# lokyhark/spalinalg

Hardware: AMD Instinct MI355X
Metric: CSR SpMV GFLOP/s (f64, 10Mx10M, 140M nnz) (higher is better)
Workload: dtype f64

## Files before the change

spalinalg_amd/csrc/csr_slide.hpp:

```cpp
#pragma once
#include "csr_kernels.hpp"

namespace spal {

constexpr uint32_t kSlideAsync = 1u << 16;
constexpr uint32_t kSlideAsyncVecs = 1;
#ifndef SPAL_SLIDE_FIRST_BATCH
#define SPAL_SLIDE_FIRST_BATCH 12
#endif
constexpr uint32_t kSlideFirstBatch = SPAL_SLIDE_FIRST_BATCH;

template <typename T>
struct SlideVec { using type = __attribute__((ext_vector_type(4))) uint32_t; };

template <typename T>
__device__ __forceinline__ typename SlideVec<T>::type slide_load_vec(const T *__restrict__ x, uint32_t page, uint32_t v,
                                                                      uint32_t last_vec) {
    using vec_t = typename SlideVec<T>::type;
    constexpr uint32_t VP = kPageCols / (16 / sizeof(T));
    return reinterpret_cast<const vec_t *>(x)[min(page * VP + v, last_vec)];
}

template <typename T>
__device__ __forceinline__ typename SlideVec<T>::type slide_load_vec_tail(const T *__restrict__ x, uint32_t page, uint32_t v,
// ... 11 lines not shown
}

struct SlideNew { uint32_t lo0, lo1, hi0, hi1; };
__device__ __forceinline__ SlideNew slide_new_pages(uint32_t fa, uint32_t na, uint32_t fb, uint32_t nb) {
    const uint32_t ea = fa + na, eb = fb + nb;
    SlideNew r;
    if (fa >= eb || ea <= fb) {
        r.lo0 = fb; r.lo1 = eb; r.hi0 = eb; r.hi1 = eb;
        return r;
    }
    r.lo0 = fb; r.lo1 = max(fb, min(fa, eb));
    r.hi0 = min(eb, max(ea, fb)); r.hi1 = eb;
    return r;
}

template <typename T, int RPT, int S, bool UNI>
__device__ __forceinline__ void slide_tile_load(StreamTile<T> &t, const uint32_t *__restrict__ rowptr,
                                                const uint16_t *__restrict__ col16, const T *__restrict__ vals,
                                                uint32_t row0, uint32_t nrows, uint32_t b, uint32_t e, uint32_t lane,
                                                uint32_t ulen) {
    using pair_t = typename Pair<T>::type;
    static_assert(RPT <= 64, "a row per lane");
    const uint32_t rlast = min(row0 + (uint32_t)RPT, nrows);
    t.start = b & ~1u;
    t.steps = (e - t.start + 127u) >> 7;
    const uint32_t e0 = t.start + lane * 2;
    const uint32_t jmax = max(t.steps, 1u) - 1u;
#pragma unroll
    for (int j = 0; j < S; ++j) {
        const uint32_t at = e0 + min((uint32_t)j, jmax) * 128u;
        t.v[j] = __builtin_nontemporal_load(reinterpret_cast<const pair_t *>(vals + at));
        t.c[j] = __builtin_nontemporal_load(reinterpret_cast<const uint32_t *>(col16 + at));
    }
    if constexpr (UNI) {
        const uint32_t len = ulen - 1u, nrt = rlast - min(row0, rlast);
        t.rp0 = b + min(lane, nrt) * len;
        t.rp1 = b + min(lane + 1u, nrt) * len;
    } else {
        t.rp0 = rowptr[min(row0 + lane, rlast)];
        t.rp1 = rowptr[min(row0 + lane + 1u, rlast)];
    }
}

template <typename T, int RPT, int S, bool UNI, int PF>
__global__ __launch_bounds__(kStreamBlock, 2) void csr_spmv_slide(
    const uint32_t *__restrict__ rowptr, const uint16_t *__restrict__ col16, const T *__restrict__ vals,
    const T *__restrict__ x, T *__restrict__ y, const uint2 *__restrict__ sdesc, uint32_t nrows, uint32_t ncols,
    uint32_t nsteps, uint32_t per_xcd, uint32_t chunk, uint32_t NP, uint32_t ulen, uint32_t flags) {
    static_assert(PF == 1 || PF == 2, "one or two tiles of loads ahead");
    static_assert(S >= 1 && S <= kStreamSteps, "a tile holds at most kStreamSteps steps");
    using vec_t = typename SlideVec<T>::type;
    extern __shared__ __attribute__((aligned(16))) unsigned char spal_smem[];
    constexpr uint32_t V = 16 / sizeof(T), VP = kPageCols / V;
    constexpr int NB = PF + 1;
    const bool nt_store = flags & 1u;
    T *prod_all = reinterpret_cast<T *>(spal_smem);
    T *xw = prod_all + kStreamWaves * stream_strip<false>();
    vec_t *xw4 = reinterpret_cast<vec_t *>(xw);

    const uint32_t xcd = blockIdx.x & 7u, slot = blockIdx.x >> 3, slots = gridDim.x >> 3;
    const bool even = flags & 8u;
    const uint32_t xbase = even ? xcd * (nsteps / 8u) + min(xcd, nsteps % 8u) : xcd * per_xcd;
    if (xbase >= nsteps) return;
    const uint32_t nx = even ? nsteps / 8u + (xcd < nsteps % 8u ? 1u : 0u) : min(per_xcd, nsteps - xbase);
    if (nx == 0u) return;
// ... 18 lines not shown
    const bool arith = UNI && (flags & 4u);
    auto tile_b = [&](uint32_t k) { const uint32_t r = min(tile_row(k), nrows); return arith ? r * (ulen - 1u) : rowptr[r]; };
    auto tile_e = [&](uint32_t k) { const uint32_t r = min(tile_row(k) + (uint32_t)RPT, nrows); return arith ? r * (ulen - 1u) : rowptr[r]; };

    StreamTile<T> t[NB];
    uint32_t tb[NB], te[NB];
#pragma unroll
    for (int q = 0; q < NB; ++q) {
        tb[q] = tile_b((uint32_t)q);
        te[q] = tile_e((uint32_t)q);
    }
    uint2 d = sdesc[gi(0u)];
    uint2 dn = sdesc[gi(1u)];
#pragma unroll
    for (int q = 0; q < PF; ++q)
        slide_tile_load<T, RPT, S, UNI>(t[q], rowptr, col16, vals, tile_row((uint32_t)q), nrows, tb[q], te[q], lane, ulen);
    {
        const uint32_t f = d.x, nv = (d.y & 0xffu) * VP;
        for (uint32_t j0 = threadIdx.x; j0 < nv; j0 += kSlideFirstBatch * kStreamBlock) {
            vec_t r[kSlideFirstBatch];
#pragma unroll
            for (uint32_t k = 0; k < kSlideFirstBatch; ++k) {
                const uint32_t j = min(j0 + k * kStreamBlock, nv - 1u);
                r[k] = slide_load_vec_tail<T>(x, f + j / VP, j % VP, ncols);
            }
#pragma unroll
            for (uint32_t k = 0; k < kSlideFirstBatch; ++k) {
                const uint32_t j = j0 + k * kStreamBlock;
                if (j < nv) xw4[((f + j / VP) % NP) * VP + j % VP] = r[k];
            }
        }
// ... 5 lines not shown
        constexpr int KN = (K + PF) % NB;
        const uint32_t skip = (d.y >> 8) & 0xfu;
        const bool more = i + 1u < nk;
        SlideNew nw = slide_new_pages(d.x, d.y & 0xffu, dn.x, dn.y & 0xffu);
        const uint32_t nlo = (nw.lo1 - nw.lo0) * VP;
        const uint32_t ntot = more ? nlo + (nw.hi1 - nw.hi0) * VP : 0u;
        const bool async = more && (dn.y & kSlideAsync) && (even || (i + 1u) % chunk != 0u);
        auto new_page = [&](uint32_t j) { return j < nlo ? nw.lo0 + j / VP : nw.hi0 + (j - nlo) / VP; };
        vec_t nv[kSlideAsyncVecs];
#pragma unroll
        for (uint32_t k = 0; k < kSlideAsyncVecs; ++k) {
            const uint32_t j = threadIdx.x + k * kStreamBlock;
            const bool mine = async && j < ntot;
            nv[k] = slide_load_vec<T>(x, mine ? new_page(j) : 0u, mine ? j % VP : 0u, last_vec);
        }
        slide_tile_load<T, RPT, S, UNI>(t[KN], rowptr, col16, vals, tile_row(i + PF), nrows, tb[KN], te[KN], lane, ulen);
        tb[K] = tile_b(i + PF + 1u);
        te[K] = tile_e(i + PF + 1u);
        const uint32_t r0 = (gi(i) * kStreamWaves + wave) * (uint32_t)RPT;
#ifdef SPAL_DIAG
        if (SPAL_DIAG_ON(flags, 11)) {
            T sacc = T(0);
#pragma unroll
            for (int j = 0; j < S; ++j) sacc += t[K].v[j].x + t[K].v[j].y + T(t[K].c[j]);
            if (r0 + lane < nrows) y[r0 + lane] = sacc + T(t[K].rp1 - t[K].rp0);
        } else
#endif
        if (r0 < nrows && !((skip >> wave) & 1u)) {
            stream_compute<T, RPT, false>(t[K], xw, wmax, prod, y, r0, nrows, lane, nt_store, flags);
        } else if (r0 < nrows && ((d.y >> (20u + wave)) & 1u)) {
            const uint32_t re = min(r0 + (uint32_t)RPT, nrows), rm = min(r0 + (uint32_t)RPT / 2u, re);
            const uint32_t eb = rowptr[r0], em = rowptr[rm], ee = rowptr[re];
            slide_tile_load<T, RPT, S, false>(t[K], rowptr, col16, vals, r0, rm, eb, em, lane, 0u);
            stream_compute<T, RPT, false>(t[K], xw, wmax, prod, y, r0, rm, lane, nt_store, flags);
            if (rm < re) {
                __builtin_amdgcn_wave_barrier();
                slide_tile_load<T, RPT, S, false>(t[K], rowptr, col16, vals, rm, re, em, ee, lane, 0u);
                stream_compute<T, RPT, false>(t[K], xw, wmax, prod, y, rm, re, lane, nt_store, flags);
            }
        }
#pragma unroll
        for (uint32_t k = 0; k < kSlideAsyncVecs; ++k) {
            const uint32_t j = threadIdx.x + k * kStreamBlock;
            if (async && j < ntot) xw4[(new_page(j) % NP) * VP + j % VP] = nv[k];
        }
// ... 31 lines not shown
```

spalinalg_amd/csrc/spal_csr.hip:

```cpp
#include "csr_kernels.hpp"
#include "csr_slide.hpp"
#include "spal_ops.hpp"

namespace spal {

template <typename K>
static hipError_t raise_lds_cap(K kern, int device, size_t lds, std::atomic<uint64_t> &configured) {
    if (lds <= 48 * 1024) return hipSuccess;
    const uint64_t bit = 1ull << (device & 63);
    if (configured.load(std::memory_order_relaxed) & bit) return hipSuccess;
    hipError_t e = hipFuncSetAttribute((const void *)kern, hipFuncAttributeMaxDynamicSharedMemorySize,
                                       160 * 1024);
    if (e == hipSuccess) configured.fetch_or(bit, std::memory_order_relaxed);
    return e;
}

template <typename T, int L, int U, bool LDSX, int BLOCK, int LB = 1>
static hipError_t launch_vec(const spal_csr *a, const void *x, void *y, hipStream_t st) {
    const CsrPlan &p = a->plan;
    const uint32_t per_xcd = (p.nblocks + 7) / 8;
    const size_t lds = LDSX ? (size_t)p.lds_entries * sizeof(T) : 0;
    auto kern = csr_spmv_vector<T, L, U, LDSX, true, BLOCK, LB>;
    static std::atomic<uint64_t> configured{0};
    hipError_t e = raise_lds_cap(kern, a->device, lds, configured);
// ... 231 lines not shown
    const hipError_t e = typed([&](auto t) { return launch_lanes<decltype(t)>(a, x_dev, y_dev, stream); });
    if (e != hipSuccess)
        return fail(SPAL_ERR_HIP, "csr spmv launch failed: %s", hipGetErrorString(e));
    return SPAL_OK;
}

void csr_free(spal_csr *a) {
    if (!a) return;
    for (spal_csr *part : a->parts) csr_free(part);
    (void)dev_free(a->d_rowptr);
    (void)dev_free(a->d_colind);
    (void)dev_free(a->d_values);
    (void)dev_free(a->d_desc);
    if (a->col16_placed) place_free(a->device, a->d_col16);
    else (void)dev_free(a->d_col16);
    (void)dev_free(a->d_pages);
    (void)dev_free(a->d_ovtiles);
    (void)dev_free(a->d_sdesc);
    (void)dev_free(a->d_ovtiles_slide);
    (void)dev_free(a->d_ptiles);
    (void)dev_free(a->d_pwin);
    if (a->split_short) csr_free(a->split_short);
    (void)dev_free(a->d_split_rows);
    blockwin_free(a);
    if (a->d_vec_block && a->vec_block_owned) (void)hipFree(a->d_vec_block);
    else place_free(a->device, a->d_vec_block);
    (void)dev_free(a->d_win_groups);
    cblock_free(a);
    trsv_free(a);
    trsv_sweep_free(a);
// ... 288 lines not shown
    {"stream_global", &CsrPlan::stream_global, 0, 1, nullptr, "stream_global must be 0 or 1"},
    {"window_pages", &CsrPlan::window_pages, 0, 64, nullptr, "window_pages must be in [0, 64]"},
    {"col16", &CsrPlan::vec_col16_allowed, 0, 1, nullptr, "col16 must be 0 or 1"},
    {"stream_row_max", &CsrPlan::stream_row_max, 1, 1024, nullptr, "stream_row_max must be in [1, 1024]"},
    {"nt_store", &CsrPlan::nt_store, 0, 1, nullptr, "nt_store must be 0 or 1"},
    {"persistent_blocks", &CsrPlan::persistent_blocks, 0, 4096, [](int64_t v) { return v == 0 || (v >= 8 && v % 8 == 0); },
     "persistent_blocks must be 0 (auto) or a multiple of 8 in [8, 4096]"},
    {"slide", &CsrPlan::slide_user, -1, 1, nullptr, "slide must be -1 (auto), 0 or 1"},
    {"panel_pages", &CsrPlan::panel_pages, 0, 255, nullptr, "panel_pages must be in [0, 255]"},
    {"panel_window", &CsrPlan::panel_window_user, 0, 624, nullptr, "panel_window must be in [0, 624] pages"},
    {"panel_on", &CsrPlan::panel_on, 0, 1, nullptr, "panel_on must be 0 or 1"},
    {"slide_run", &CsrPlan::slide_run, 0, 65535, nullptr, "slide_run must be in [0, 65535]"},
    {"slide_even", &CsrPlan::slide_even, 0, 1, nullptr, "slide_even must be 0 or 1"},
    {"arith_bounds", &CsrPlan::arith_bounds, 0, 1, nullptr, "arith_bounds must be 0 or 1"},
    {"split_tiles", &CsrPlan::split_tiles_on, 0, 1, nullptr, "split_tiles must be 0 or 1"},
    {"place_tries", &CsrPlan::place_tries, 0, 16, nullptr, "place_tries must be in [0, 16]"},
    {"uniform_rows", &CsrPlan::uniform_rows, 0, 1, nullptr, "uniform_rows must be 0 or 1"},
    {"prefetch", &CsrPlan::prefetch, 1, 2, nullptr, "prefetch must be 1 or 2"},
    {"xcd_chunk", &CsrPlan::xcd_chunk, 0, 4096, nullptr, "xcd_chunk must be in [0, 4096]"},
    {"cblock_rows", &CsrPlan::cblock_rows_user, 0, 8192, nullptr,
     "cblock_rows (rows of a row block of the column-blocked kernel) must be 0 (auto) or in [1, 8192]"},
    {"cblock_shift", &CsrPlan::cblock_shift_user, 0, 24, [](int64_t v) { return v == 0 || v >= 8; },
     "cblock_shift (log2 of the columns of a column block) must be 0 (auto: 2 MB of x) or in [8, 24]"},
    {"cblock_form", &CsrPlan::cblock_form_user, -1, 1, nullptr, "cblock_form must be -1 (auto), 0 (entry-parallel) or 1 (rows form)"},
};

int spal_csr_set_option(spal_csr_t a, const char *key, int64_t value) {
    if (!a || !key) return fail(SPAL_ERR_INVALID_ARGUMENT, "spal_csr_set_option: null argument");
    {
        int st = SPAL_OK;
// ... 180 lines not shown
             (p.kernel == 2 && p.persistent && p.tiles_per_wave == 4) ? 1 : 0,
             p.kernel == 2 ? p.nt_store : 0, p.kernel == 2 ? p.uniform_row_fraction : 0.0,
             p.kernel == 2 ? p.prefetch : 0, (p.kernel == 2 && p.slide && p.slide_on && p.slide_fill_ok) ? 1 : 0,
             p.kernel == 2 ? p.ring_pages : 0, (p.kernel == 2 && p.slide) ? p.slide_S : 0,
             (p.kernel == 2 && p.slide && p.slide_on) ? a->n_split_tiles : 0u,
             (p.kernel == 2 && p.panel_on) ? a->n_ptiles : 0u,
             (double)a->tuned_us[0], (double)a->tuned_us[1],
             (double)a->tuned_us[2], (double)a->tuned_us[3], (double)a->place_us[0], (double)a->place_us[1],
             a->place_tried, (unsigned long long)(uintptr_t)a->d_values,
             (unsigned long long)(uintptr_t)a->d_col16, (unsigned long long)(uintptr_t)a->d_rowptr,
             (double)a->walk_us[0], (double)a->walk_us[1], a->walk_blocks, a->walk_probes, place_block_count(a->device),
             (unsigned long long)place_free_bytes(a->device),
             p.kernel == 2 ? p.nonlocal_row_fraction : 0.0, (p.cblock && p.cblock_on) ? 1 : 0, p.cblock_pending, p.cblock ? p.cblock_rows : 0, !p.cblock ? "" : p.cblock_form ? "rows" : "entry", p.cblock ? (double)p.cblock_run : 0.0,
             p.cblock ? (1ull << p.cblock_shift) : 0ull, p.cblock ? p.cblock_nbc : 0, p.cblock ? p.cblock_nrb : 0u,
             (double)a->cblock_us[0], (double)a->cblock_us[1], a->cblock_failed);
    return SPAL_OK;
}
int spal_csr_describe(spal_csr_t a, char *buf, size_t buf_len) {
    if (!a || !buf || !buf_len) return fail(SPAL_ERR_INVALID_ARGUMENT, "spal_csr_describe: null argument");
    SPAL_TRY(csr_describe_plan(a, buf, buf_len));
    return ops_describe_append(buf, buf_len, a->ops, a);
}

}
```

spalinalg_amd/csrc/spal_csr_plan.hip:

```cpp
#include "csr_kernels.hpp"
#include "spal_internal.hpp"

namespace spal {

__global__ __launch_bounds__(256) void csr_block_windows(
    const uint32_t *__restrict__ rowptr, const uint32_t *__restrict__ colind, uint32_t nrows,
    uint32_t R, uint2 *__restrict__ out) {
    __shared__ uint32_t s_min, s_max;
    if (threadIdx.x == 0) {
        s_min = 0xffffffffu;
        s_max = 0u;
    }
    __syncthreads();
    const uint32_t row0 = blockIdx.x * R;
    const uint32_t row1 = min(row0 + R, nrows);
    uint32_t lo = 0xffffffffu, hi = 0u;
    for (uint32_t r = row0 + threadIdx.x; r < row1; r += 256) {
        const uint32_t a0 = rowptr[r], a1 = rowptr[r + 1];
        if (a0 < a1) {
            lo = min(lo, colind[a0]);
            hi = max(hi, colind[a1 - 1] + 1u);
        }
    }
    atomicMin(&s_min, lo);
// ... 425 lines not shown
        }
    }
    CsrPlan &p = a->plan;
    const double mean = a->nrows ? (double)a->nnz / (double)a->nrows : 0.0;
    if (!p.user_lanes) p.lanes_per_row = mean > 85.0 ? 64 : mean > 64.0 ? 32 : pick_lanes(mean);
    p.long_rows = mean > 64.0 ? 1 : 0;
    if (!p.user_unroll) p.unroll = mean > 64.0 ? 1 : 4;
    if (!p.user_threads) p.threads = 1024;
    if (a->d_desc) {
        SPAL_HIP_TRY(dev_free(a->d_desc));
        a->d_desc = nullptr;
    }
    p.stream_row_fraction = 0.0;
    p.vec_col16 = 0;
    p.slide = 0;
    p.ring_pages = 0;
    if (a->nnz == 0) {
        cblock_free(a);
        p.kernel = 1;
        p.rows_per_block = 1024;
        p.nblocks = (uint32_t)((a->nrows + 1023) / 1024);
        p.lds_x = 0;
        return SPAL_OK;
    }
    const uint32_t valign = 16u / (uint32_t)a->elem_size;

    if ((p.user_kernel == 0 && mean <= 120.0) || p.user_kernel == 2) {
        if (p.tiles_per_wave != 4 && p.tiles_per_wave != 8) p.tiles_per_wave = 4;
        const int rpt_all[] = {256, 128, 64, 32, 24, 16, 12, 8};
        std::vector<int> rpts;
// ... 87 lines not shown
            for (uint32_t b = 0; b < p.nblocks && !any_stream; ++b) any_stream = best_desc[b].z == kModeStream;
            if (any_stream || a->n_ptiles) {
                if (!a->d_col16) {
                    SPAL_HIP_TRY(dev_alloc((void **)&a->d_col16, (size_t)a->cap_entries * sizeof(uint16_t)));
                    SPAL_HIP_TRY(hipMemsetAsync(a->d_col16, 0, (size_t)a->cap_entries * sizeof(uint16_t), a->stream));
                }
                if (any_stream)
                    hipLaunchKernelGGL(csr_encode_col16, dim3(p.nblocks), dim3(256), 0, a->stream, a->d_rowptr,
                                       a->d_colind, a->d_desc, a->d_pages, a->d_col16, (uint32_t)a->nrows, R,
                                       (uint32_t)p.ring_pages);
                if (a->n_ptiles)
                    hipLaunchKernelGGL(csr_encode_col16_span, dim3(a->n_ptiles), dim3(256), 0, a->stream, a->d_rowptr,
                                       a->d_colind, a->d_ptiles, a->d_pwin, a->d_col16, (uint32_t)a->nrows, R);
                SPAL_HIP_TRY(hipGetLastError());
            }
            if (best_over) {
                uint32_t *d_list = nullptr;
                const uint32_t pieces = (uint32_t)std::max(1, best_rpt / 64) * best_over;
                SPAL_HIP_TRY(dev_alloc((void **)&d_list, ((size_t)pieces + 1) * 4));
                a->d_ovtiles = d_list;
                SPAL_HIP_TRY(hipMemsetAsync(d_list, 0, 4, a->stream));
                const uint64_t ntile = (a->nrows + (uint64_t)best_rpt - 1) / (uint64_t)best_rpt;
                hipLaunchKernelGGL(csr_overflow_tiles, dim3((uint32_t)((ntile + 255) / 256)), dim3(256), 0, a->stream,
                                   a->d_desc, (uint32_t)a->nrows, R, (uint32_t)best_rpt, pieces, d_list,
                                   d_list + 1);
                SPAL_HIP_TRY(hipGetLastError());
                uint32_t listed = 0;
                SPAL_HIP_TRY(hipMemcpyAsync(&listed, d_list, 4, hipMemcpyDeviceToHost, a->stream));
                SPAL_HIP_TRY(hipStreamSynchronize(a->stream));
                if (listed > pieces || listed < best_over)
// ... 9 lines not shown
                p.nonlocal_row_fraction = (double)far_rows / (double)a->nrows;
                p.cblock_pending = 0;
                if (getenv("SPAL_CBLOCK_DEBUG"))
                    fprintf(stderr, "[spal cblock] plan: nonlocal rows %.3f, user %d, lazy %d\n", p.nonlocal_row_fraction, p.cblock_user, a->cblock_lazy);
                if (p.cblock_user == 1 || (p.cblock_user < 0 && p.nonlocal_row_fraction >= 0.5)) {
                    if (a->cblock_lazy && p.cblock_user < 0) { cblock_free(a); p.cblock_pending = 1; }
                    else (void)cblock_plan(a, p.cblock_user == 1);
                } else {
                    cblock_free(a);
                }
            }
            return SPAL_OK;
        }
    }
    cblock_free(a);

    p.kernel = 1;
    if (p.threads != 512 && p.threads != 1024) p.threads = 1024;
    const uint32_t budget = kLdsBudgetBytes / (uint32_t)a->elem_size;
    const uint32_t cand_all[] = {4096, 2048, 1024, 512};
    std::vector<uint32_t> cands;
    if (p.user_rows_per_block) {
        cands.push_back((uint32_t)p.rows_per_block);
    } else if (mean > 64.0) {
        uint32_t r0 = 1024;
        while (r0 > 64 && (double)r0 * mean > 131072.0) r0 >>= 1;
        if (p.threads == 1024) {
            const double want = std::max(1.0, (double)a->nnz / 100000.0);
            const uint64_t rounds = std::max<uint64_t>(1, (uint64_t)(want / 512.0 + 0.5));
            const uint64_t nb = rounds * 502;
// ... 71 lines not shown
```

spalinalg_amd/csrc/spal_csr_slide.hip:

```cpp
#include "csr_panel.hpp"
#include "csr_slide.hpp"
#include "spal_internal.hpp"

namespace spal {

template <typename T, int RPT, int S, bool UNI>
static hipError_t launch_slide_inst(const spal_csr *a, const void *x, void *y, hipStream_t st) {
    constexpr int PF = 2;
    const CsrPlan &p = a->plan;
    const size_t lds = ((size_t)kStreamWaves * stream_strip<false>() + (size_t)p.ring_pages * kPageCols) * sizeof(T);
    const int per_cu = (int)std::min<size_t>(8, std::max<size_t>(1, (160 * 1024) / (lds + 512)));
    const uint32_t grid = p.persistent_blocks > 0 ? (uint32_t)p.persistent_blocks : 256u * (uint32_t)per_cu;
    const uint32_t per_xcd = (p.slide_steps + 7u) / 8u;
    const uint32_t slots = std::max(1u, grid / 8u);
    const uint32_t one_run = (per_xcd + slots - 1u) / slots;
    const uint32_t chunk = p.slide_run > 0 ? std::min<uint32_t>((uint32_t)p.slide_run, one_run) : one_run;
    const bool even = p.slide_run <= 0 && p.slide_even;
    const uint32_t used = even ? std::min(slots, per_xcd) : std::min(slots, (per_xcd + chunk - 1u) / chunk);
    auto kern = csr_spmv_slide<T, RPT, S, UNI, PF>;
    static std::atomic<uint64_t> configured{0};
    const uint64_t bit = 1ull << (a->device & 63);
    if (lds > 48 * 1024 && !(configured.load(std::memory_order_relaxed) & bit)) {
        hipError_t e = hipFuncSetAttribute((const void *)kern, hipFuncAttributeMaxDynamicSharedMemorySize, 160 * 1024);
        if (e != hipSuccess) return e;
        configured.fetch_or(bit, std::memory_order_relaxed);
    }
    hipLaunchKernelGGL(kern, dim3(used * 8u), dim3(kStreamBlock), lds, st, a->d_rowptr, a->d_col16,
                       (const T *)a->d_values, (const T *)x, (T *)y, a->d_sdesc, (uint32_t)a->nrows, (uint32_t)a->ncols,
                       p.slide_steps, per_xcd, chunk, (uint32_t)p.ring_pages, (uint32_t)p.slide_uniform,
                       (uint32_t)(p.nt_store ? 1 : 0) | (uint32_t)p.diag | ((UNI && p.all_rows_uniform && p.arith_bounds) ? 4u : 0u) | (even ? 8u : 0u));
    return hipGetLastError();
}

template <typename T, int RPT, bool UNI>
static hipError_t launch_slide_steps(const spal_csr *a, const void *x, void *y, hipStream_t st) {
    switch (std::max(4, a->plan.slide_S)) {
        case 4: return launch_slide_inst<T, RPT, 4, UNI>(a, x, y, st);
        case 5: return launch_slide_inst<T, RPT, 5, UNI>(a, x, y, st);
        case 6: return launch_slide_inst<T, RPT, 6, UNI>(a, x, y, st);
        case 7: return launch_slide_inst<T, RPT, 7, UNI>(a, x, y, st);
        case 8: return launch_slide_inst<T, RPT, 8, UNI>(a, x, y, st);
        default: return hipErrorInvalidValue;
// ... 7 lines not shown
}

template <typename T>
static hipError_t launch_slide_rpt(const spal_csr *a, const void *x, void *y, hipStream_t st) {
    switch (a->plan.rows_per_tile) {
        case 64: return launch_slide_uni<T, 64>(a, x, y, st);
        case 32: return launch_slide_uni<T, 32>(a, x, y, st);
        case 24: return launch_slide_uni<T, 24>(a, x, y, st);
        case 16: return launch_slide_uni<T, 16>(a, x, y, st);
        case 12: return launch_slide_uni<T, 12>(a, x, y, st);
        case 8: return launch_slide_uni<T, 8>(a, x, y, st);
        default: return hipErrorInvalidValue;
    }
}

hipError_t launch_slide(const spal_csr *a, const void *x, void *y, hipStream_t st) {
    return a->elem_size == 8 ? launch_slide_rpt<double>(a, x, y, st) : launch_slide_rpt<float>(a, x, y, st);
}

template <typename T, int RPT>
static hipError_t launch_panel_inst(const spal_csr *a, const void *x, void *y, hipStream_t st) {
    const CsrPlan &p = a->plan;
    const size_t lds = std::max((size_t)kStreamWaves * stream_strip<false>(), (size_t)p.panel_window_pages * kPageCols) * sizeof(T);
    auto kern = csr_spmv_panel<T, RPT>;
    static std::atomic<uint64_t> configured{0};
    const uint64_t bit = 1ull << (a->device & 63);
    if (lds > 48 * 1024 && !(configured.load(std::memory_order_relaxed) & bit)) {
        hipError_t e = hipFuncSetAttribute((const void *)kern, hipFuncAttributeMaxDynamicSharedMemorySize, 160 * 1024);
        if (e != hipSuccess) return e;
        configured.fetch_or(bit, std::memory_order_relaxed);
    }
// ... 142 lines not shown
    p.slide = 1;
    p.ring_pages = (int)NP;
    p.slide_steps = nsteps;
    p.slide_S = (int)S;
    p.slide_uniform = (uni && ulen != 0u) ? (int)ulen : 0;
    {
        const double tiles = (double)nsteps * kStreamWaves;
        const double avg_steps = tiles > 0 ? (double)a->nnz / tiles / 128.0 : 0.0;
        p.slide_fill_ok = (p.slide_fill_user >= 0) ? p.slide_fill_user : (avg_steps >= 0.6 * (double)std::max(4u, S) ? 1 : 0);
    }
    p.all_rows_uniform = (p.slide_uniform && left_over.empty() && n_split == 0 &&
                          (uint64_t)a->nrows * (uint64_t)(ulen - 1u) == a->nnz) ? 1 : 0;
    return SPAL_OK;
}

}
```

spalinalg_amd/csrc/spal_csr_tune.hip:

```cpp
#include "spal_internal.hpp"

namespace spal {

template <typename T>
static int csr_autotune(spal_csr_t a, const T *x_dev, T *y_dev, void *stream, int iters) {
    if (!a) return fail(SPAL_ERR_INVALID_ARGUMENT, "spal_csr_autotune: handle is NULL");
    if (a->elem_size != (int)sizeof(T))
        return fail(SPAL_ERR_INVALID_ARGUMENT, "spal_csr_autotune: handle holds %s values",
                    a->elem_size == 8 ? "f64" : "f32");
    if (!x_dev || !y_dev) return fail(SPAL_ERR_INVALID_ARGUMENT, "spal_csr_autotune: null vector");
    if (!a->parts.empty()) {
        for (size_t b = 0; b < a->parts.size(); ++b)
            SPAL_TRY(csr_autotune<T>(a->parts[b], x_dev, y_dev + a->part_row0[b], stream, iters));
        return SPAL_OK;
    }
    if (iters < 1) iters = 1;
    DeviceGuard guard(a->device);
    if (guard.status != SPAL_OK) return guard.status;
    SPAL_TRY(csr_ensure_plan(a, nullptr, false));
    if (a->bw_on) return SPAL_OK;
    if (a->split_short) return csr_autotune<T>(a->split_short, x_dev, y_dev, stream, iters);
    std::lock_guard<std::mutex> lock(a->mu);
    CsrPlan &p = a->plan;
    for (float &t : a->tuned_us) t = 0.f;
// ... 38 lines not shown
            p.nt_store = (cand >> 1) & 1;
            float ms = 0.f;
            timed(iters, &ms);
            if (rc == SPAL_OK && round == 1) {
                a->tuned_us[cand] = ms * 1e3f;
                if (ms < best_ms) { best_ms = ms; best = cand; }
                if (cand == planned) planned_ms = ms;
            }
        }
    }
    if (planned_ms <= 1.01f * best_ms) best = planned;
    if (walking_is_slide) { p.slide_on = best & 1; p.slide_fill_ok = 1; p.persistent = 0; }
    else p.persistent = best & 1;
    p.user_persistent = true;
    p.nt_store = (best >> 1) & 1;
    int tries = p.place_tries;
    if (const char *e = getenv("SPAL_PLACE_TRIES")) tries = atoi(e);
    const size_t cbytes = a->d_col16 ? (size_t)a->cap_entries * sizeof(uint16_t) : 0;
    if (rc == SPAL_OK && tries > 0 && cbytes >= ((size_t)64 << 20) && !a->col16_placed) {
        const int n = std::max(4, iters / 4);
        float cur_ms = 0.f;
        timed(n, &cur_ms);
        a->place_us[0] = cur_ms * 1e3f;
        uint16_t *const original = a->d_col16;
        std::vector<void *> cand;
        std::vector<float> ms_of;
        const int kept = place_block_count(a->device);
        for (int k = 0; k < kept && k < tries && rc == SPAL_OK; ++k) {
            void *b = place_alloc(a->device, k, cbytes);
            if (!b) continue;
            hipError_t e = hipMemcpyAsync(b, original, cbytes, hipMemcpyDeviceToDevice, st);
            if (e != hipSuccess) { place_free(a->device, b); rc = fail(SPAL_ERR_HIP, "spal_csr_autotune: %s", hipGetErrorString(e)); break; }
            a->d_col16 = (uint16_t *)b;
            float ms = 0.f;
            timed(n, &ms);
            cand.push_back(b); ms_of.push_back(ms);
            ++a->place_tried;
        }
        int best = -1;
        for (size_t k = 0; k < ms_of.size(); ++k)
            if (ms_of[k] < 0.99f * cur_ms && (best < 0 || ms_of[k] < ms_of[(size_t)best])) best = (int)k;
        (void)hipStreamSynchronize(st);
        a->d_col16 = best >= 0 ? (uint16_t *)cand[(size_t)best] : original;
        for (size_t k = 0; k < cand.size(); ++k)
            if ((int)k != best) place_free(a->device, cand[k]);
        if (best >= 0) { (void)dev_free(original); a->col16_placed = 1; }
        a->place_us[1] = (best >= 0 ? ms_of[(size_t)best] : cur_ms) * 1e3f;
    }
    return rc;
}

}

using namespace spal;

extern "C" {

int spal_csr_alloc_vectors(spal_csr_t a, void **x_dev, void **y_dev, void *stream) {
    if (!a || !x_dev || !y_dev) return fail(SPAL_ERR_INVALID_ARGUMENT, "spal_csr_alloc_vectors: null argument");
    DeviceGuard guard(a->device);
    if (guard.status != SPAL_OK) return guard.status;
// ... 127 lines not shown
```

spalinalg_amd/csrc/spal_internal.hpp:

```cpp
#pragma once

#include <hip/hip_runtime.h>
#include <stdint.h>

#include <algorithm>
#include <atomic>
#include <cstdarg>
#include <cstdio>
#include <cstring>
#include <functional>
#include <mutex>
#include <string>
#include <thread>
#include <vector>

#include "../../include/spal.h"

namespace spal {

std::string &last_error_ref();
int fail(int status, const char *fmt, ...) __attribute__((format(printf, 2, 3)));

#define SPAL_HIP_TRY(expr)                                                          \
    do {                                                                            \
// ... 155 lines not shown
    int cblock_rows_user = 0, cblock_shift_user = 0;
    int cblock_form_user = -1;
    int cblock_form = 0;
    float cblock_run = 0.f;
    int cblock_shift = 0;
    int cblock_nbc = 0;
    uint32_t cblock_nrb = 0;
    double nonlocal_row_fraction = 0.0;
    int slide_S = 0;
    int slide_uniform = 0;
    int all_rows_uniform = 0;
    int arith_bounds = 1;
    int slide_fill_ok = 1;
    int slide_fill_user = -1;
    int slide_even = 1;
    int blockwin = -1;
    int row_split = -1;
    int split_threshold = 128;
    int place_tries = 8;
    int split_tiles_on = 1;
    int diag = 0;
    int persistent_blocks = 0;
    int rows_per_block = 0;
    int lds_x = 0;
    uint32_t lds_entries = 0;
    uint32_t nblocks = 0;
    double lds_row_fraction = 0.0;
    double stream_row_fraction = 0.0;
    double uniform_row_fraction = 0.0;
    bool user_rows_per_block = false, user_lanes = false, user_lds = false,
// ... 86 lines not shown
    uint32_t bw_blocks = 0, bw_rows = 0, bw_cols = 0, bw_grid = 0;
    uint32_t bw_list_rows = 0;
    int bw_on = 0;
    float bw_us[2] = {0.f, 0.f};
    int plan_pending = 0;
    int cblock_lazy = 0;
    int cblock_failed = 0;
    void *d_vec_block = nullptr;
    int vec_block_owned = 0;
    size_t vec_x_off = 0, vec_y_off = 0;
    float walk_us[2] = {0.f, 0.f};
    int walk_blocks = 0;
    int walk_probes = 0;
    int walk_max = 8;
    int col16_placed = 0;
    std::mutex mu_cb;
    float tuned_us[4] = {0.f, 0.f, 0.f, 0.f};
    float place_us[2] = {0.f, 0.f};
    int place_tried = 0;
    spal::CsrPlan plan;
    std::vector<uint2> win_base;
    uint2 *d_win_groups = nullptr;
    uint32_t win_groups = 0, win_group_bits = 0;
    std::mutex mu;
    void *d_x = nullptr, *d_y = nullptr;
    hipStream_t stream = nullptr;
    std::vector<spal_csr *> parts;
    std::vector<uint64_t> part_row0, part_entry0;
    spal::OpState ops;
    uint64_t spmm_last = 0;
// ... 90 lines not shown
namespace spal {
int csr_plan_build(spal_csr *a);
constexpr uint32_t kWinBase = 256;
int csr_try_row_split(spal_csr *a, bool *did);
int csr_blockwin_or_split(spal_csr *a);
int csr_launch(spal_csr *a, const void *x_dev, void *y_dev, hipStream_t stream);
int csr_launch_planned(spal_csr *a, const void *x_dev, void *y_dev, hipStream_t stream);
int csr_ensure_plan(spal_csr *a, hipStream_t launch_stream, bool from_launch);
void csr_free(spal_csr *a);
int spmm_launch(spal_csr *a, int tile, uint64_t k, const void *x_dev, uint64_t ldx, void *y_dev, uint64_t ldy,
                hipStream_t stream);
void trsv_free(spal_csr *a);
void trsv_sweep_free(spal_csr *a);
hipError_t launch_slide(const spal_csr *a, const void *x, void *y, hipStream_t st);
int slide_plan(spal_csr *a, uint32_t rpt, const std::vector<uint4> &desc, const std::vector<uint32_t> &skip, uint32_t super_pages);
hipError_t launch_panel(const spal_csr *a, const void *x, void *y, hipStream_t st);
int csc_plan_build(spal_csc *a);
constexpr uint32_t kCscModeGlobal = 0, kCscModeLds = 1;
constexpr uint32_t kCscChunk = 1024;
hipError_t launch_csc_scatter(spal_csc *a, const void *x, void *y, hipStream_t st);
uint32_t csc_window_budget(const spal_csc *a, int cols);
size_t csc_scatter_lds_bytes(const spal_csc *a);
int csc_scatter_per_cu(const spal_csc *a);
bool csc_gave_up_consume(spal_csc *a);
int csc_invalid_products(const spal_csc *a);
int csc_rowtiles_plan(spal_csc *a);
void csc_rowtiles_free(spal_csc *a);
hipError_t launch_csc_rowtiles(const spal_csc *a, const void *x, void *y, hipStream_t st);
int cblock_plan(spal_csr *a, bool force);
void cblock_free(spal_csr *a);
// ... 11 lines not shown
```

Measured before the change: 1158.

## Compress uniform-row column indices into packed per-row delta records for slide SpMV

For matrices whose rows all have the same even length (12–16), each row's ring-relative column positions are encoded at plan time as a base plus byte deltas and a high-bit mask in 5–6 dwords per row. The slide kernel loads these records instead of the 16-bit column array, then decodes them in registers and transposes them through LDS into the usual tile column layout. This is meant to cut column-index traffic, roughly 24 bytes per row instead of 28–32, since SpMV is bandwidth bound. In exchange it adds decode ALU work, extra LDS round-trips and wave barriers per tile, plus build and verify kernels at planning time. The path is auto-enabled and then kept or dropped by an autotune timing comparison.

```diff
diff --git a/spalinalg_amd/csrc/csr_rowrec.hpp b/spalinalg_amd/csrc/csr_rowrec.hpp
--- /dev/null
+++ b/spalinalg_amd/csrc/csr_rowrec.hpp
@@ -0,0 +1,101 @@
+#pragma once
+#include <stdint.h>
+
+#if defined(__HIPCC__)
+#define SPAL_ROWREC_HD __host__ __device__ __forceinline__
+#else
+#define SPAL_ROWREC_HD inline
+#endif
+
+namespace spal {
+
+constexpr int kRowrecMinLen = 12, kRowrecMaxLen = 16;
+constexpr int kRowrecHighBits = 40;
+constexpr int kRowrecMaxDwords = 6;
+constexpr int rowrec_dwords(int L) { return L <= 14 ? 5 : 6; }
+constexpr bool rowrec_length_ok(int L) { return L >= kRowrecMinLen && L <= kRowrecMaxLen && L % 2 == 0; }
+constexpr uint32_t rowrec_max_span(int L, uint32_t R) {
+    const uint32_t by_bits = ((uint32_t)(kRowrecHighBits - 1 - (L - 2)) << 8) | 255u;
+    return R == 0u ? 0u : (by_bits < R - 1u ? by_bits : R - 1u);
+}
+
+template <int L>
+SPAL_ROWREC_HD void rowrec_pad(uint32_t *rec) {
+    const uint64_t H = (1ull << (L - 1)) - 1ull;
+    rec[0] = (uint32_t)(H << 16);
+    rec[1] = (uint32_t)(H >> 16);
+    for (int q = 2; q < rowrec_dwords(L); ++q) rec[q] = 0u;
+}
+
+template <int L>
+SPAL_ROWREC_HD bool rowrec_encode(const uint32_t *cols, uint32_t R, uint32_t *rec) {
+    static_assert(L >= 2 && L - 1 <= kRowrecHighBits && 7 + L - 1 <= 4 * kRowrecMaxDwords, "the record's fields");
+    constexpr int NR = rowrec_dwords(L);
+    for (int k = 1; k < L; ++k)
+        if (cols[k] <= cols[k - 1]) return false;
+    const uint32_t span = cols[L - 1] - cols[0];
+    if (R == 0u || R > 65536u || span >= R || (span >> 8) + (uint32_t)(L - 2) > (uint32_t)(kRowrecHighBits - 1)) return false;
+    uint64_t H = 0;
+    uint32_t w[kRowrecMaxDwords] = {0u, 0u, 0u, 0u, 0u, 0u};
+    for (int k = 1; k < L; ++k) {
+        const uint32_t d = cols[k] - cols[0];
+        H |= 1ull << ((d >> 8) + (uint32_t)(k - 1));
+        const int byte = 7 + (k - 1);
+        w[byte >> 2] |= (d & 255u) << (8 * (byte & 3));
+    }
+    w[0] |= (cols[0] % R) | (uint32_t)(H << 16);
+    w[1] |= (uint32_t)(H >> 16);
+    for (int q = 0; q < NR; ++q) rec[q] = w[q];
+    return true;
+}
+
+template <int L>
+SPAL_ROWREC_HD void rowrec_decode(const uint32_t *rec, uint32_t R, uint32_t *pos) {
+    const uint32_t base = rec[0] & 0xffffu;
+    uint64_t H = (uint64_t)(rec[0] >> 16) | ((uint64_t)(rec[1] & 0xffffffu) << 16);
+    pos[0] = base;
+#if defined(__clang__)
+#pragma unroll
+#endif
+    for (int k = 1; k < L; ++k) {
+        const uint32_t b = (uint32_t)__builtin_ctzll(H | (1ull << kRowrecHighBits));
+        H &= H - 1ull;
+        const int byte = 7 + (k - 1);
+        const uint32_t low = (rec[byte >> 2] >> (8 * (byte & 3))) & 255u;
+        const uint32_t p = base + (((b - (uint32_t)(k - 1)) << 8) | low);
+        pos[k] = p >= R ? p - R : p;
+    }
+}
+
+}
+
+#if defined(__HIPCC__)
+#include "csr_kernels.hpp"
+
+namespace spal {
+
+template <typename T, int L>
+__device__ __forceinline__ void rowrec_tile_load(StreamTile<T> &t, const uint32_t *__restrict__ rec, uint32_t tix,
+                                                 uint32_t lane) {
+    constexpr int NR = rowrec_dwords(L);
+    const uint32_t *at = rec + (size_t)tix * (NR * 64u) + lane;
+#pragma unroll
+    for (int q = 0; q < NR; ++q) t.c[q] = __builtin_nontemporal_load(at + q * 64);
+}
+
+template <typename T, int L>
+__device__ __forceinline__ void rowrec_expand(StreamTile<T> &t, uint32_t *strip, uint32_t R, uint32_t lane) {
+    static_assert(L % 2 == 0 && L / 2 <= kStreamSteps && 64 * (L / 2) * 4 <= kStreamTileNnz * (int)sizeof(T), "the strip holds the tile");
+    uint32_t pos[L];
+    rowrec_decode<L>(t.c, R, pos);
+    __builtin_amdgcn_wave_barrier();
+#pragma unroll
+    for (int i = 0; i < L / 2; ++i) strip[(L / 2) * lane + i] = pos[2 * i] | (pos[2 * i + 1] << 16);
+    __builtin_amdgcn_wave_barrier();
+#pragma unroll
+    for (int j = 0; j < L / 2; ++j) t.c[j] = strip[j * 64 + lane];
+    __builtin_amdgcn_wave_barrier();
+}
+
+}
+#endif
diff --git a/spalinalg_amd/csrc/csr_slide.hpp b/spalinalg_amd/csrc/csr_slide.hpp
--- a/spalinalg_amd/csrc/csr_slide.hpp
+++ b/spalinalg_amd/csrc/csr_slide.hpp
@@ -1,5 +1,6 @@
 #pragma once
 #include "csr_kernels.hpp"
+#include "csr_rowrec.hpp"
 
 namespace spal {
 
@@ -49,7 +50,7 @@
     return r;
 }
 
-template <typename T, int RPT, int S, bool UNI>
+template <typename T, int RPT, int S, bool UNI, int REC = 0>
 __device__ __forceinline__ void slide_tile_load(StreamTile<T> &t, const uint32_t *__restrict__ rowptr,
                                                 const uint16_t *__restrict__ col16, const T *__restrict__ vals,
                                                 uint32_t row0, uint32_t nrows, uint32_t b, uint32_t e, uint32_t lane,
@@ -61,11 +62,12 @@
     t.steps = (e - t.start + 127u) >> 7;
     const uint32_t e0 = t.start + lane * 2;
     const uint32_t jmax = max(t.steps, 1u) - 1u;
+    if constexpr (REC != 0) rowrec_tile_load<T, REC>(t, reinterpret_cast<const uint32_t *>(col16), row0 / 64u, lane);
 #pragma unroll
     for (int j = 0; j < S; ++j) {
         const uint32_t at = e0 + min((uint32_t)j, jmax) * 128u;
         t.v[j] = __builtin_nontemporal_load(reinterpret_cast<const pair_t *>(vals + at));
-        t.c[j] = __builtin_nontemporal_load(reinterpret_cast<const uint32_t *>(col16 + at));
+        if constexpr (REC == 0) t.c[j] = __builtin_nontemporal_load(reinterpret_cast<const uint32_t *>(col16 + at));
     }
     if constexpr (UNI) {
         const uint32_t len = ulen - 1u, nrt = rlast - min(row0, rlast);
@@ -77,13 +79,14 @@
     }
 }
 
-template <typename T, int RPT, int S, bool UNI, int PF>
+template <typename T, int RPT, int S, bool UNI, int PF, int REC = 0>
 __global__ __launch_bounds__(kStreamBlock, 2) void csr_spmv_slide(
     const uint32_t *__restrict__ rowptr, const uint16_t *__restrict__ col16, const T *__restrict__ vals,
     const T *__restrict__ x, T *__restrict__ y, const uint2 *__restrict__ sdesc, uint32_t nrows, uint32_t ncols,
     uint32_t nsteps, uint32_t per_xcd, uint32_t chunk, uint32_t NP, uint32_t ulen, uint32_t flags) {
     static_assert(PF == 1 || PF == 2, "one or two tiles of loads ahead");
     static_assert(S >= 1 && S <= kStreamSteps, "a tile holds at most kStreamSteps steps");
+    static_assert(REC == 0 || (UNI && RPT == 64 && rowrec_length_ok(REC) && S == REC / 2), "row records: uniform rows, a row per lane");
     using vec_t = typename SlideVec<T>::type;
     extern __shared__ __attribute__((aligned(16))) unsigned char spal_smem[];
     constexpr uint32_t V = 16 / sizeof(T), VP = kPageCols / V;
@@ -132,7 +135,7 @@
     uint2 dn = sdesc[gi(1u)];
 #pragma unroll
     for (int q = 0; q < PF; ++q)
-        slide_tile_load<T, RPT, S, UNI>(t[q], rowptr, col16, vals, tile_row((uint32_t)q), nrows, tb[q], te[q], lane, ulen);
+        slide_tile_load<T, RPT, S, UNI, REC>(t[q], rowptr, col16, vals, tile_row((uint32_t)q), nrows, tb[q], te[q], lane, ulen);
     {
         const uint32_t f = d.x, nv = (d.y & 0xffu) * VP;
         for (uint32_t j0 = threadIdx.x; j0 < nv; j0 += kSlideFirstBatch * kStreamBlock) {
@@ -168,7 +171,7 @@
             const bool mine = async && j < ntot;
             nv[k] = slide_load_vec<T>(x, mine ? new_page(j) : 0u, mine ? j % VP : 0u, last_vec);
         }
-        slide_tile_load<T, RPT, S, UNI>(t[KN], rowptr, col16, vals, tile_row(i + PF), nrows, tb[KN], te[KN], lane, ulen);
+        slide_tile_load<T, RPT, S, UNI, REC>(t[KN], rowptr, col16, vals, tile_row(i + PF), nrows, tb[KN], te[KN], lane, ulen);
         tb[K] = tile_b(i + PF + 1u);
         te[K] = tile_e(i + PF + 1u);
         const uint32_t r0 = (gi(i) * kStreamWaves + wave) * (uint32_t)RPT;
@@ -181,8 +184,9 @@
         } else
 #endif
         if (r0 < nrows && !((skip >> wave) & 1u)) {
+            if constexpr (REC != 0) rowrec_expand<T, REC>(t[K], reinterpret_cast<uint32_t *>(prod), NP * kPageCols, lane);
             stream_compute<T, RPT, false>(t[K], xw, wmax, prod, y, r0, nrows, lane, nt_store, flags);
-        } else if (r0 < nrows && ((d.y >> (20u + wave)) & 1u)) {
+        } else if (REC == 0 && r0 < nrows && ((d.y >> (20u + wave)) & 1u)) {
             const uint32_t re = min(r0 + (uint32_t)RPT, nrows), rm = min(r0 + (uint32_t)RPT / 2u, re);
             const uint32_t eb = rowptr[r0], em = rowptr[rm], ee = rowptr[re];
             slide_tile_load<T, RPT, S, false>(t[K], rowptr, col16, vals, r0, rm, eb, em, lane, 0u);
diff --git a/spalinalg_amd/csrc/spal_csr.hip b/spalinalg_amd/csrc/spal_csr.hip
--- a/spalinalg_amd/csrc/spal_csr.hip
+++ b/spalinalg_amd/csrc/spal_csr.hip
@@ -269,6 +269,7 @@
     (void)dev_free(a->d_desc);
     if (a->col16_placed) place_free(a->device, a->d_col16);
     else (void)dev_free(a->d_col16);
+    rowrec_free(a);
     (void)dev_free(a->d_pages);
     (void)dev_free(a->d_ovtiles);
     (void)dev_free(a->d_sdesc);
@@ -587,6 +588,8 @@
     {"slide_even", &CsrPlan::slide_even, 0, 1, nullptr, "slide_even must be 0 or 1"},
     {"arith_bounds", &CsrPlan::arith_bounds, 0, 1, nullptr, "arith_bounds must be 0 or 1"},
     {"split_tiles", &CsrPlan::split_tiles_on, 0, 1, nullptr, "split_tiles must be 0 or 1"},
+    {"rowrec", &CsrPlan::rowrec_user, -1, 1, nullptr, "rowrec must be -1 (auto), 0 or 1"},
+    {"rowrec_on", &CsrPlan::rowrec_on, 0, 1, nullptr, "rowrec_on must be 0 or 1"},
     {"place_tries", &CsrPlan::place_tries, 0, 16, nullptr, "place_tries must be in [0, 16]"},
     {"uniform_rows", &CsrPlan::uniform_rows, 0, 1, nullptr, "uniform_rows must be 0 or 1"},
     {"prefetch", &CsrPlan::prefetch, 1, 2, nullptr, "prefetch must be 1 or 2"},
@@ -797,6 +800,19 @@
              p.kernel == 2 ? p.nonlocal_row_fraction : 0.0, (p.cblock && p.cblock_on) ? 1 : 0, p.cblock_pending, p.cblock ? p.cblock_rows : 0, !p.cblock ? "" : p.cblock_form ? "rows" : "entry", p.cblock ? (double)p.cblock_run : 0.0,
              p.cblock ? (1ull << p.cblock_shift) : 0ull, p.cblock ? p.cblock_nbc : 0, p.cblock ? p.cblock_nrb : 0u,
              (double)a->cblock_us[0], (double)a->cblock_us[1], a->cblock_failed);
+    if (p.kernel == 2 && p.slide) {
+        const bool rr = p.rowrec && a->d_rowrec;
+        const int rr_len = p.slide_uniform - 1;
+        SPAL_TRY(describe_append(buf, buf_len, "rowrec", rr ? "1" : "0"));
+        SPAL_TRY(describe_append(buf, buf_len, "rowrec_on", (rr && p.rowrec_on && p.slide_on && p.slide_fill_ok) ? "1" : "0"));
+        SPAL_TRY(describe_append(buf, buf_len, "rowrec_bytes_per_row", std::to_string(rr ? 4 * rowrec_dwords(p.rowrec) : 0)));
+        SPAL_TRY(describe_append(buf, buf_len, "rowrec_max_span",
+                                 std::to_string(rowrec_length_ok(rr_len) ? rowrec_max_span(rr_len, (uint32_t)p.ring_pages * kPageCols) : 0u)));
+        SPAL_TRY(describe_append(buf, buf_len, "rowrec_failed", std::to_string(p.rowrec_failed)));
+        char us[64];
+        snprintf(us, sizeof(us), "[%.1f, %.1f]", (double)a->rowrec_us[0], (double)a->rowrec_us[1]);
+        SPAL_TRY(describe_append(buf, buf_len, "rowrec_us", us));
+    }
     return SPAL_OK;
 }
 int spal_csr_describe(spal_csr_t a, char *buf, size_t buf_len) {
diff --git a/spalinalg_amd/csrc/spal_csr_plan.hip b/spalinalg_amd/csrc/spal_csr_plan.hip
--- a/spalinalg_amd/csrc/spal_csr_plan.hip
+++ b/spalinalg_amd/csrc/spal_csr_plan.hip
@@ -463,6 +463,7 @@
     p.stream_row_fraction = 0.0;
     p.vec_col16 = 0;
     p.slide = 0;
+    p.rowrec = 0;
     p.ring_pages = 0;
     if (a->nnz == 0) {
         cblock_free(a);
@@ -580,6 +581,7 @@
                                        a->d_colind, a->d_ptiles, a->d_pwin, a->d_col16, (uint32_t)a->nrows, R);
                 SPAL_HIP_TRY(hipGetLastError());
             }
+            SPAL_TRY(rowrec_plan(a));
             if (best_over) {
                 uint32_t *d_list = nullptr;
                 const uint32_t pieces = (uint32_t)std::max(1, best_rpt / 64) * best_over;
@@ -619,6 +621,7 @@
         }
     }
     cblock_free(a);
+    rowrec_free(a);
 
     p.kernel = 1;
     if (p.threads != 512 && p.threads != 1024) p.threads = 1024;
diff --git a/spalinalg_amd/csrc/spal_csr_slide.hip b/spalinalg_amd/csrc/spal_csr_slide.hip
--- a/spalinalg_amd/csrc/spal_csr_slide.hip
+++ b/spalinalg_amd/csrc/spal_csr_slide.hip
@@ -4,7 +4,7 @@
 
 namespace spal {
 
-template <typename T, int RPT, int S, bool UNI>
+template <typename T, int RPT, int S, bool UNI, int REC = 0>
 static hipError_t launch_slide_inst(const spal_csr *a, const void *x, void *y, hipStream_t st) {
     constexpr int PF = 2;
     const CsrPlan &p = a->plan;
@@ -17,7 +17,8 @@
     const uint32_t chunk = p.slide_run > 0 ? std::min<uint32_t>((uint32_t)p.slide_run, one_run) : one_run;
     const bool even = p.slide_run <= 0 && p.slide_even;
     const uint32_t used = even ? std::min(slots, per_xcd) : std::min(slots, (per_xcd + chunk - 1u) / chunk);
-    auto kern = csr_spmv_slide<T, RPT, S, UNI, PF>;
+    auto kern = csr_spmv_slide<T, RPT, S, UNI, PF, REC>;
+    const uint16_t *cols = REC != 0 ? reinterpret_cast<const uint16_t *>(a->d_rowrec) : a->d_col16;
     static std::atomic<uint64_t> configured{0};
     const uint64_t bit = 1ull << (a->device & 63);
     if (lds > 48 * 1024 && !(configured.load(std::memory_order_relaxed) & bit)) {
@@ -25,7 +26,7 @@
         if (e != hipSuccess) return e;
         configured.fetch_or(bit, std::memory_order_relaxed);
     }
-    hipLaunchKernelGGL(kern, dim3(used * 8u), dim3(kStreamBlock), lds, st, a->d_rowptr, a->d_col16,
+    hipLaunchKernelGGL(kern, dim3(used * 8u), dim3(kStreamBlock), lds, st, a->d_rowptr, cols,
                        (const T *)a->d_values, (const T *)x, (T *)y, a->d_sdesc, (uint32_t)a->nrows, (uint32_t)a->ncols,
                        p.slide_steps, per_xcd, chunk, (uint32_t)p.ring_pages, (uint32_t)p.slide_uniform,
                        (uint32_t)(p.nt_store ? 1 : 0) | (uint32_t)p.diag | ((UNI && p.all_rows_uniform && p.arith_bounds) ? 4u : 0u) | (even ? 8u : 0u));
@@ -63,7 +64,18 @@
     }
 }
 
+template <typename T>
+static hipError_t launch_slide_rowrec(const spal_csr *a, const void *x, void *y, hipStream_t st) {
+    switch (a->plan.rowrec) {
+        case 12: return launch_slide_inst<T, 64, 6, true, 12>(a, x, y, st);
+        case 14: return launch_slide_inst<T, 64, 7, true, 14>(a, x, y, st);
+        case 16: return launch_slide_inst<T, 64, 8, true, 16>(a, x, y, st);
+        default: return hipErrorInvalidValue;
+    }
+}
+
 hipError_t launch_slide(const spal_csr *a, const void *x, void *y, hipStream_t st) {
+    if (rowrec_runs(a)) return a->elem_size == 8 ? launch_slide_rowrec<double>(a, x, y, st) : launch_slide_rowrec<float>(a, x, y, st);
     return a->elem_size == 8 ? launch_slide_rpt<double>(a, x, y, st) : launch_slide_rpt<float>(a, x, y, st);
 }
 
@@ -236,4 +248,97 @@
     return SPAL_OK;
 }
 
-}
+template <int L>
+__global__ __launch_bounds__(256) void rowrec_build(const uint32_t *__restrict__ colind, uint32_t nrows, uint32_t rows_padded,
+                                                    uint32_t R, uint32_t *__restrict__ rec, uint32_t *__restrict__ flag) {
+    constexpr int NR = rowrec_dwords(L);
+    const uint32_t r = blockIdx.x * 256u + threadIdx.x;
+    if (r >= rows_padded) return;
+    uint32_t w[kRowrecMaxDwords];
+    rowrec_pad<L>(w);
+    if (r < nrows) {
+        uint32_t cols[L];
+#pragma unroll
+        for (int k = 0; k < L; ++k) cols[k] = colind[(size_t)r * L + k];
+        if (!rowrec_encode<L>(cols, R, w)) atomicOr(&flag[0], 1u);
+    }
+    uint32_t *at = rec + (size_t)(r / 64u) * (NR * 64u) + r % 64u;
+#pragma unroll
+    for (int q = 0; q < NR; ++q) at[q * 64] = w[q];
+}
+
+template <int L>
+__global__ __launch_bounds__(256) void rowrec_verify(const uint32_t *__restrict__ rec, const uint16_t *__restrict__ col16,
+                                                     uint32_t nrows, uint32_t R, uint32_t *__restrict__ flag) {
+    constexpr int NR = rowrec_dwords(L);
+    const uint32_t r = blockIdx.x * 256u + threadIdx.x;
+    if (r >= nrows) return;
+    uint32_t w[kRowrecMaxDwords] = {0u, 0u, 0u, 0u, 0u, 0u}, pos[L];
+    const uint32_t *at = rec + (size_t)(r / 64u) * (NR * 64u) + r % 64u;
+#pragma unroll
+    for (int q = 0; q < NR; ++q) w[q] = at[q * 64];
+    rowrec_decode<L>(w, R, pos);
+    bool same = true;
+#pragma unroll
+    for (int k = 0; k < L; ++k) same = same && pos[k] == (uint32_t)col16[(size_t)r * L + k];
+    if (!same) atomicOr(&flag[1], 1u);
+}
+
+void rowrec_free(spal_csr *a) {
+    if (a->rowrec_placed) place_free(a->device, a->d_rowrec);
+    else (void)dev_free(a->d_rowrec);
+    a->d_rowrec = nullptr;
+    a->rowrec_bytes = 0;
+    a->rowrec_placed = 0;
+}
+
+int rowrec_plan(spal_csr *a) {
+    CsrPlan &p = a->plan;
+    p.rowrec = 0;
+    p.rowrec_failed = 0;
+    const int L = p.slide_uniform - 1;
+    if (p.rowrec_user == 0 || !p.slide || !p.all_rows_uniform || !p.arith_bounds || p.rows_per_tile != 64 ||
+        p.tiles_per_wave != 4 || !rowrec_length_ok(L) || p.slide_S != L / 2 || !a->d_col16) {
+        rowrec_free(a);
+        return SPAL_OK;
+    }
+    const uint32_t R = (uint32_t)p.ring_pages * kPageCols;
+    const uint32_t rows_padded = p.slide_steps * 256u;
+    const size_t bytes = (size_t)p.slide_steps * 4u * (size_t)rowrec_dwords(L) * 64u * sizeof(uint32_t);
+    if (a->d_rowrec && a->rowrec_bytes != bytes) rowrec_free(a);
+    if (!a->d_rowrec) {
+        if (dev_alloc((void **)&a->d_rowrec, bytes) != hipSuccess) {
+            (void)hipGetLastError();
+            a->d_rowrec = nullptr;
+            return SPAL_OK;
+        }
+        a->rowrec_bytes = bytes;
+    }
+    DevBuf d_flag;
+    SPAL_HIP_TRY(d_flag.alloc(2 * sizeof(uint32_t)));
+    SPAL_HIP_TRY(hipMemsetAsync(d_flag.p, 0, 2 * sizeof(uint32_t), a->stream));
+    const dim3 gb((rows_padded + 255u) / 256u), gv((uint32_t)((a->nrows + 255) / 256));
+    auto run = [&](auto len) {
+        constexpr int LL = decltype(len)::value;
+        hipLaunchKernelGGL(rowrec_build<LL>, gb, dim3(256), 0, a->stream, a->d_colind, (uint32_t)a->nrows, rows_padded, R,
+                           a->d_rowrec, d_flag.as<uint32_t>());
+        hipLaunchKernelGGL(rowrec_verify<LL>, gv, dim3(256), 0, a->stream, a->d_rowrec, a->d_col16, (uint32_t)a->nrows, R,
+                           d_flag.as<uint32_t>());
+    };
+    if (L == 12) run(std::integral_constant<int, 12>{});
+    else if (L == 14) run(std::integral_constant<int, 14>{});
+    else run(std::integral_constant<int, 16>{});
+    SPAL_HIP_TRY(hipGetLastError());
+    uint32_t flag[2] = {0u, 0u};
+    SPAL_HIP_TRY(hipMemcpyAsync(flag, d_flag.p, sizeof(flag), hipMemcpyDeviceToHost, a->stream));
+    SPAL_HIP_TRY(hipStreamSynchronize(a->stream));
+    if (flag[0] || flag[1]) {
+        rowrec_free(a);
+        p.rowrec_failed = (!flag[0] && flag[1]) ? 1 : 0;
+        return SPAL_OK;
+    }
+    p.rowrec = L;
+    return SPAL_OK;
+}
+
+}
diff --git a/spalinalg_amd/csrc/spal_csr_tune.hip b/spalinalg_amd/csrc/spal_csr_tune.hip
--- a/spalinalg_amd/csrc/spal_csr_tune.hip
+++ b/spalinalg_amd/csrc/spal_csr_tune.hip
@@ -76,15 +76,28 @@
     else p.persistent = best & 1;
     p.user_persistent = true;
     p.nt_store = (best >> 1) & 1;
+    a->rowrec_us[0] = a->rowrec_us[1] = 0.f;
+    if (rc == SPAL_OK && walking_is_slide && p.slide_on && p.rowrec && a->d_rowrec) {
+        float ms[2] = {0.f, 0.f};
+        for (int round = 0; round < 2 && rc == SPAL_OK; ++round)
+            for (int on = 0; on < 2 && rc == SPAL_OK; ++on) { p.rowrec_on = on; timed(iters, &ms[on]); }
+        if (rc == SPAL_OK) {
+            a->rowrec_us[0] = ms[0] * 1e3f; a->rowrec_us[1] = ms[1] * 1e3f;
+            p.rowrec_on = ms[1] <= 0.99f * ms[0] ? 1 : 0;
+        }
+    }
     int tries = p.place_tries;
     if (const char *e = getenv("SPAL_PLACE_TRIES")) tries = atoi(e);
-    const size_t cbytes = a->d_col16 ? (size_t)a->cap_entries * sizeof(uint16_t) : 0;
-    if (rc == SPAL_OK && tries > 0 && cbytes >= ((size_t)64 << 20) && !a->col16_placed) {
+    const bool recs = rowrec_runs(a) && walking_is_slide && p.slide_on;
+    void **const slot = recs ? (void **)&a->d_rowrec : (void **)&a->d_col16;
+    int *const placed = recs ? &a->rowrec_placed : &a->col16_placed;
+    const size_t cbytes = recs ? a->rowrec_bytes : a->d_col16 ? (size_t)a->cap_entries * sizeof(uint16_t) : 0;
+    if (rc == SPAL_OK && tries > 0 && cbytes >= ((size_t)64 << 20) && !*placed) {
         const int n = std::max(4, iters / 4);
         float cur_ms = 0.f;
         timed(n, &cur_ms);
         a->place_us[0] = cur_ms * 1e3f;
-        uint16_t *const original = a->d_col16;
+        void *const original = *slot;
         std::vector<void *> cand;
         std::vector<float> ms_of;
         const int kept = place_block_count(a->device);
@@ -93,7 +106,7 @@
             if (!b) continue;
             hipError_t e = hipMemcpyAsync(b, original, cbytes, hipMemcpyDeviceToDevice, st);
             if (e != hipSuccess) { place_free(a->device, b); rc = fail(SPAL_ERR_HIP, "spal_csr_autotune: %s", hipGetErrorString(e)); break; }
-            a->d_col16 = (uint16_t *)b;
+            *slot = b;
             float ms = 0.f;
             timed(n, &ms);
             cand.push_back(b); ms_of.push_back(ms);
@@ -103,10 +116,10 @@
         for (size_t k = 0; k < ms_of.size(); ++k)
             if (ms_of[k] < 0.99f * cur_ms && (best < 0 || ms_of[k] < ms_of[(size_t)best])) best = (int)k;
         (void)hipStreamSynchronize(st);
-        a->d_col16 = best >= 0 ? (uint16_t *)cand[(size_t)best] : original;
+        *slot = best >= 0 ? cand[(size_t)best] : original;
         for (size_t k = 0; k < cand.size(); ++k)
             if ((int)k != best) place_free(a->device, cand[k]);
-        if (best >= 0) { (void)dev_free(original); a->col16_placed = 1; }
+        if (best >= 0) { (void)dev_free(original); *placed = 1; }
         a->place_us[1] = (best >= 0 ? ms_of[(size_t)best] : cur_ms) * 1e3f;
     }
     return rc;
diff --git a/spalinalg_amd/csrc/spal_internal.hpp b/spalinalg_amd/csrc/spal_internal.hpp
--- a/spalinalg_amd/csrc/spal_internal.hpp
+++ b/spalinalg_amd/csrc/spal_internal.hpp
@@ -193,6 +193,10 @@
     int slide_fill_ok = 1;
     int slide_fill_user = -1;
     int slide_even = 1;
+    int rowrec_user = -1;
+    int rowrec_on = 1;
+    int rowrec = 0;
+    int rowrec_failed = 0;
     int blockwin = -1;
     int row_split = -1;
     int split_threshold = 128;
@@ -309,6 +313,10 @@
     int walk_probes = 0;
     int walk_max = 8;
     int col16_placed = 0;
+    uint32_t *d_rowrec = nullptr;
+    size_t rowrec_bytes = 0;
+    int rowrec_placed = 0;
+    float rowrec_us[2] = {0.f, 0.f};
     std::mutex mu_cb;
     float tuned_us[4] = {0.f, 0.f, 0.f, 0.f};
     float place_us[2] = {0.f, 0.f};
@@ -429,6 +437,9 @@
 void trsv_sweep_free(spal_csr *a);
 hipError_t launch_slide(const spal_csr *a, const void *x, void *y, hipStream_t st);
 int slide_plan(spal_csr *a, uint32_t rpt, const std::vector<uint4> &desc, const std::vector<uint32_t> &skip, uint32_t super_pages);
+int rowrec_plan(spal_csr *a);
+void rowrec_free(spal_csr *a);
+inline bool rowrec_runs(const spal_csr *a) { return a->plan.rowrec && a->plan.rowrec_on && a->d_rowrec; }
 hipError_t launch_panel(const spal_csr *a, const void *x, void *y, hipStream_t st);
 int csc_plan_build(spal_csc *a);
 constexpr uint32_t kCscModeGlobal = 0, kCscModeLds = 1;
```

Measured after the change: 1203 (median of 6 runs). +3.8%, better.
